# JeongsooP/RGB-no-more

Hardware: AMD Instinct MI355X
Metric: images/sec JPEG-Ti DCT 512x512 train step (higher is better)
Workload: dtype bf16

## Files before the change

rgb-no-more_amd/csrc/vit_chain_bwd.hip:

```cpp
#include "common.h"
#include <string.h>
#include <type_traits>
#include "internal.h"
#include "ln_bwd_rows.h"
#include "../../include/rgbnm.h"

namespace {

typedef __attribute__((address_space(3))) void* lds_ptr;
typedef const __attribute__((address_space(1))) void* glb_ptr;
typedef unsigned int u32x2 __attribute__((ext_vector_type(2)));
typedef unsigned int u32x4 __attribute__((ext_vector_type(4)));
typedef bf16 bf16x2v __attribute__((ext_vector_type(2)));

constexpr int E = 192, HID = 768, HD = 64, HEADS = 3, NTOK = 196, NTILE = 7, NPAD = 224, INNER = HEADS * HD, LDQ = 3 * INNER;
constexpr int NCW = 7, NTHREADS = 64 * (NCW + 1), CTHREADS = 64 * NCW, BM = 32 * NCW;
constexpr int ROWB = 128, ARR = NPAD * ROWB, SLOT = 24576, STAGE = 2 * SLOT, CH = 64, NCHUNK = HID / CH;
constexpr int CP = E + 4;
constexpr int SMEM = 163840;
#ifndef PIPE_P
#define PIPE_P 6
#endif
#ifndef PIPE_M1
#define PIPE_M1 5
#endif
#ifndef PIPE_X
#define PIPE_X 7
#endif
constexpr int M_STG = 2 * STAGE;
constexpr int TILE = 32 * ROWB;
typedef rgbnm::LnBwdRows<CTHREADS, BM> LnBwd;
constexpr int RED_OFF = (BM * CP * 2 + 1023) / 1024 * 1024;
static_assert(RED_OFF + LnBwd::RED_BYTES <= 132096, "LDS");
constexpr int P_SLOT0 = 132096, P_SLOT1 = 0, P_TILES = 98304;
static_assert(P_SLOT0 + SLOT <= SMEM && P_TILES + NCW * TILE <= P_SLOT0, "LDS");
constexpr int A_Q = 0, A_K = ARR, A_V = 2 * ARR, A_G = 3 * ARR, A_L2 = 4 * ARR, A_D = A_L2 + NPAD * 4, A_STG = A_D + NPAD * 4;
constexpr int STG_PITCH = 144, STG_WAVE = 32 * STG_PITCH;
constexpr int A_SIDE = A_STG + NCW * STG_WAVE;
static_assert(A_SIDE + NCW * 1024 <= SMEM, "LDS");
constexpr int X_SLOT0 = A_K, X_SLOT1 = A_K + SLOT, X_SLOT2 = 0, X_TILES = A_K + 2 * SLOT, X_TSET = NCW * TILE;
static_assert(X_SLOT1 + SLOT <= X_TILES && X_TILES + 3 * X_TSET <= SMEM && SLOT <= A_K, "LDS");

struct BwdBlk {
  const bf16* wimg;
  const float *ln1_g, *ln2_g;
  const bf16* x_in; const float *mean1, *rstd1;
  const bf16* qkv; const float* lse; const bf16* attn; const bf16* x_mid; const float *mean2, *rstd2; const bf16* gp;
  const bf16* dy;
  bf16* du; bf16* dx_mid; bf16* dqkv; bf16* dx;
  float *part2, *part1;
};
static_assert(sizeof(BwdBlk) == sizeof(rgbnm_chain_bwd_block), "rgbnm_chain_bwd_block layout");
constexpr int MAX_DEPTH = 12;
struct BwdArgs {
  BwdBlk blk[MAX_DEPTH]; bf16* dattn;
  int depth, nimg;
  float scale;
};

__device__ __forceinline__ int fswz(int row) {
  return (((row >> 1) & 1) << 2) | ((row >> 2) & 1) | (((row >> 3) & 1) << 1);
}
struct Geo {
  int lane, l31, g, fl;
  unsigned tr0;
};
__device__ __forceinline__ Geo make_geo() {
  Geo L;
  L.lane = threadIdx.x & 63;
  L.l31 = L.lane & 31;
  L.g = L.lane >> 5;
  L.fl = fswz(L.l31);
  const int k = (L.lane >> 2) & 3, G1 = (L.lane >> 4) & 1, l3 = L.lane & 3;
  const int pc = (2 * G1 + (l3 >> 1)) ^ (((k >> 1) << 2) | L.g);
  L.tr0 = (unsigned)((4 * L.g + k) * ROWB + pc * 16 + 8 * (l3 & 1));
  return L;
}
__device__ __forceinline__ Geo fresh_geo() {
  Geo L;
  L.lane = lane_id_here();
  L.l31 = L.lane & 31;
  L.g = L.lane >> 5;
  L.fl = fswz(L.l31);
  const int k = (L.lane >> 2) & 3, G1 = (L.lane >> 4) & 1, l3 = L.lane & 3;
  const int pc = (2 * G1 + (l3 >> 1)) ^ (((k >> 1) << 2) | L.g);
  L.tr0 = (unsigned)((4 * L.g + k) * ROWB + pc * 16 + 8 * (l3 & 1));
  return L;
}
template <int T> struct TileLoop {
// ... 46 lines not shown
#ifndef XB_ROWPIPE
#define XB_ROWPIPE 1
#endif
__device__ __forceinline__ void row_pair_mma(f32x16& sa, f32x16& da, const unsigned char* arrS, const unsigned char* arrD, unsigned rb,
                                             int t, const Frag<bf16> (&xs)[4], const Frag<bf16> (&xd)[4]) {
#if XB_ROWPIPE
#define XB_SB __builtin_amdgcn_sched_barrier(0)
  Frag<bf16> fs[4], fd[4];
  XB_SB;
  fs[0] = rowfrag_x(arrS, rb, t, 0);
  fd[0] = rowfrag_x(arrD, rb, t, 0);
  fs[1] = rowfrag_x(arrS, rb, t, 1);
  fd[1] = rowfrag_x(arrD, rb, t, 1);
  XB_SB;
  mma(sa, fs[0], xs[0]); XB_SB;
  fs[2] = rowfrag_x(arrS, rb, t, 2); XB_SB;
  mma(da, fd[0], xd[0]); XB_SB;
  fd[2] = rowfrag_x(arrD, rb, t, 2); XB_SB;
  mma(sa, fs[1], xs[1]); XB_SB;
  fs[3] = rowfrag_x(arrS, rb, t, 3); XB_SB;
  mma(da, fd[1], xd[1]); XB_SB;
  fd[3] = rowfrag_x(arrD, rb, t, 3); XB_SB;
  mma(sa, fs[2], xs[2]);
  mma(da, fd[2], xd[2]);
  mma(sa, fs[3], xs[3]);
  mma(da, fd[3], xd[3]);
  XB_SB;
#undef XB_SB
#else
#pragma unroll
  for (int c = 0; c < 4; ++c) {
    mma(sa, rowfrag_x(arrS, rb, t, c), xs[c]);
    mma(da, rowfrag_x(arrD, rb, t, c), xd[c]);
  }
#endif
}
__device__ __forceinline__ unsigned opaque(unsigned v) {
  asm volatile("" : "+v"(v));
  return v;
}
__device__ __forceinline__ void wg_barrier() {
  asm volatile("" ::: "memory");
  __builtin_amdgcn_s_barrier();
  asm volatile("" ::: "memory");
}
template <int N> __device__ __forceinline__ void wait_vm() { asm volatile("s_waitcnt vmcnt(%0)" ::"n"(N) : "memory"); }
__device__ __forceinline__ void wait_lds() { asm volatile("s_waitcnt lgkmcnt(0)" ::: "memory"); }
#ifndef XB_NT
#define XB_NT 1
#endif
#ifndef XB_NTLD
#define XB_NTLD 0
#endif
template <bool NT, typename V, typename P>
__device__ __forceinline__ void gstore(P* ptr, const V& v) {
#ifdef XB_NOSTORE
  if ((XB_NOSTORE & 1) && NT) return;
  if ((XB_NOSTORE & 2) && !NT) return;
#endif
  if constexpr (NT) __builtin_nontemporal_store(v, reinterpret_cast<V*>(ptr));
  else *reinterpret_cast<V*>(ptr) = v;
}

#ifdef X_LDSWAIT
__device__ __forceinline__ void own_tile_fence() { wait_lds(); }
#else
__device__ __forceinline__ void own_tile_fence() { asm volatile("" ::: "memory"); }
#endif
__device__ __forceinline__ unsigned pack2(float a, float b) {
  const bf16x2v v = {(bf16)a, (bf16)b};
  unsigned r = __builtin_bit_cast(unsigned, v);
  asm volatile("" : "+v"(r));
  return r;
}
__device__ __forceinline__ bf16x8 as_bf16x8(u32x4 v) { return __builtin_bit_cast(bf16x8, v); }
struct Rows { u32x4 v[12]; };

template <int NKB>
__device__ __forceinline__ void dma_linear(const unsigned char* src, unsigned char* dst, int lane) {
#pragma unroll
  for (int i = 0; i < NKB; ++i)
    __builtin_amdgcn_global_load_lds((glb_ptr)(src + i * 1024 + lane * 16), (lds_ptr)(dst + i * 1024), 16, 0, 0);
}
__device__ __forceinline__ void dma_matrix_all(const bf16* __restrict__ src, int ld, unsigned char* dst, int lane) {
#pragma unroll 4
  for (int i = 0; i < 28; ++i) {
    const int row = 8 * i + (lane >> 3), pc = lane & 7;
    const int lc = pc ^ fswz(row);
    const int srow = row < NTOK ? row : NTOK - 1;
    __builtin_amdgcn_global_load_lds((glb_ptr)(src + (size_t)srow * ld + lc * 8), (lds_ptr)(dst + i * 1024), 16, 0, (XB_NTLD & 2) ? 2 : 0);
  }
}
__device__ __forceinline__ void dma_row_tiles(const bf16* __restrict__ src, int ld, unsigned char* dst, int lane) {
#pragma unroll 4
  for (int i = 0; i < 28; ++i) {
    const int row = 8 * i + (lane >> 3), pc = lane & 7;
    const int lc = pc ^ (row & 7);
    const int srow = row < NTOK ? row : NTOK - 1;
    __builtin_amdgcn_global_load_lds((glb_ptr)(src + (size_t)srow * ld + lc * 8), (lds_ptr)(dst + i * 1024), 16, 0, 0);
  }
}

__device__ __forceinline__ void tile_out(unsigned char* smem, unsigned stg, const u32x4& p0, const u32x4& p1, const u32x4& p2,
                                         const u32x4& p3, bf16* dst, int ld, int live) {
  const int ln = lane_id_here();
  const unsigned wo = stg + (unsigned)((ln & 31) * ROWB + (((ln >> 5) ^ (ln & 7)) << 4));
  *reinterpret_cast<u32x4*>(smem + wo) = p0;
  *reinterpret_cast<u32x4*>(smem + (wo ^ 32u)) = p1;
  *reinterpret_cast<u32x4*>(smem + (wo ^ 64u)) = p2;
  *reinterpret_cast<u32x4*>(smem + (wo ^ 96u)) = p3;
  own_tile_fence();
  const int rl = ln >> 3, seg = ln & 7;
  const unsigned ro = stg + (unsigned)(rl * ROWB + ((seg ^ rl) << 4));
  bf16* gp = dst + (size_t)rl * ld + seg * 8;
  u32x4 v[4];
#pragma unroll
  for (int i = 0; i < 4; ++i) v[i] = *reinterpret_cast<const u32x4*>(smem + ro + i * 8 * ROWB);
  if (live == 32) {
#pragma unroll
    for (int i = 0; i < 4; ++i) gstore<(XB_NT & 4) != 0>(gp + (size_t)i * 8 * ld, v[i]);
  } else {
#pragma unroll
    for (int i = 0; i < 4; ++i)
      if (i * 8 + rl < live) gstore<(XB_NT & 4) != 0>(gp + (size_t)i * 8 * ld, v[i]);
  }
  own_tile_fence();
}

__device__ __forceinline__ void gemm_k192(f32x16& acc, const unsigned char* sW, int ht, const Rows& x, const Geo& L) {
  int wbase = L.l31 * (E * 2) + ((L.g ^ L.fl) << 4) + ht * 32 * (E * 2);
  asm volatile("" : "+v"(wbase));
#pragma unroll
  for (int c = 0; c < 12; ++c) {
    Frag<bf16> fb, fx;
    fb.v = *reinterpret_cast<const bf16x8*>(sW + ((wbase ^ ((c % 4) << 5)) + 128 * (c / 4)));
    fx.v = as_bf16x8(x.v[c]);
    mma(acc, fb, fx);
  }
}

template <int DEPTH>
__device__ __forceinline__ void gemm_k192x2(f32x16& a0, f32x16& a1, const unsigned char* sW, const Rows& x, const Geo& L) {
  int wb0 = L.l31 * (E * 2) + ((L.g ^ L.fl) << 4);
  asm volatile("" : "+v"(wb0));
  const int wb1 = wb0 + 32 * (E * 2);
  Frag<bf16> fb[24];
#pragma unroll
  for (int i = 0; i < 24; ++i) {
    const int c = i >> 1;
    fb[i].v = *reinterpret_cast<const bf16x8*>(sW + ((((i & 1) ? wb1 : wb0) ^ ((c % 4) << 5)) + 128 * (c / 4)));
  }
#pragma unroll
  for (int i = 0; i < 24; ++i) {
    Frag<bf16> fx;
    fx.v = as_bf16x8(x.v[i >> 1]);
    mma((i & 1) ? a1 : a0, fb[i], fx);
  }
  __builtin_amdgcn_sched_group_barrier(0x100, DEPTH, 0);
#pragma unroll
  for (int i = 0; i < 24 - DEPTH; ++i) {
    __builtin_amdgcn_sched_group_barrier(0x008, 1, 0);
    __builtin_amdgcn_sched_group_barrier(0x100, 1, 0);
  }
#pragma unroll
  for (int i = 0; i < DEPTH; ++i) __builtin_amdgcn_sched_group_barrier(0x008, 1, 0);
  __builtin_amdgcn_sched_barrier(0);
}
typedef bf16 bf16x4v __attribute__((ext_vector_type(4)));
typedef __attribute__((address_space(3))) bf16x4v* lds_b64_ptr;
__device__ __forceinline__ u32x2 tr_read(const unsigned char* smem, unsigned off) {
// ... 39 lines not shown
      v[wv][i] = PRIVATE ? *reinterpret_cast<const u32x4*>(src + wv * STG_WAVE + r * STG_PITCH + seg * 16)
                         : *reinterpret_cast<const u32x4*>(src + (wv * 32 + r) * ROWB + ((seg ^ (r & 7)) << 4));
    }
}
__device__ __forceinline__ void tiles_write(const u32x4 (&v)[NTILE][4], bf16* __restrict__ g0, size_t ld, int lane) {
  const int rl = lane >> 3, seg = lane & 7;
#pragma unroll
  for (int wv = 0; wv < NTILE; ++wv)
#pragma unroll
    for (int i = 0; i < 4; ++i) {
      const int row = wv * 32 + i * 8 + rl;
      if (row < NTOK) gstore<(XB_NT & 2) != 0>(g0 + (size_t)row * ld + seg * 8, v[wv][i]);
    }
}

#ifdef CHAINB_PROF
__device__ unsigned long long g_chainb_prof[8 * 8 * 128];
#define CP_(i)                                                                                          \
  do {                                                                                                  \
    if (ib == CHAINB_PROF_BLK && blockIdx.x < 8) {                                                      \
      const unsigned long long t_ = __builtin_amdgcn_s_memtime();                                       \
      if ((threadIdx.x & 63) == 0) g_chainb_prof[(blockIdx.x * 8 + (threadIdx.x >> 6)) * 128 + (i)] = t_; \
    }                                                                                                   \
  } while (0)
#ifndef CHAINB_PROF_BLK
#define CHAINB_PROF_BLK 6
#endif
#else
#define CP_(i) do {} while (0)
#endif
#define BAR(s) do { CP_(2 * (s)); wg_barrier(); CP_(2 * (s) + 1); } while (0)
constexpr int B_M0 = 0;
constexpr int B_E2 = 12;
constexpr int B_P = 19;
constexpr int B_A = 24;
constexpr int B_X = 37;
constexpr int B_E1 = 46;
constexpr int B_END = 53;

__device__ __forceinline__ void ln_bwd_request(LnBwd& lnb, const bf16* X, const float* mean, const float* rstd, const bf16* R, int img,
                                               int w) {
  const int tid = w * 64 + lane_id_here();
  lnb.request_x(X, E, mean, rstd, img * NTOK, NTOK, tid);
  lnb.request_res(R, E, img * NTOK, NTOK, tid);
}
template <int B0>
__device__ __forceinline__ void ln_bwd_epilogue(unsigned char* smem, const f32x16 (&acc)[6], const bf16* X, const float* mean,
                                                const float* rstd, const bf16* R, const float* gamma, bf16* DX,
                                                float* part, int img, int w, int ib) {
  const int lane_ = lane_id_here();
  const int tid = w * 64 + lane_, rloc = w * 32 + (lane_ & 31), g = lane_ >> 5;
  LnBwd lnb;
  lnb.request_x(X, E, mean, rstd, img * NTOK, NTOK, tid);
  lnb.request_res(R, E, img * NTOK, NTOK, tid);
  wait_lds();
  BAR(B0);
  bf16* Cs = reinterpret_cast<bf16*>(smem);
#pragma unroll
  for (int b = 0; b < 6; ++b)
#pragma unroll
    for (int q = 0; q < 4; ++q) {
      const int nl = 32 * b + 8 * q + 4 * g;
      const f32x4 v = {acc[b][4 * q + 0], acc[b][4 * q + 1], acc[b][4 * q + 2], acc[b][4 * q + 3]};
      store4<bf16>(Cs + rloc * CP + nl, v);
    }
  wait_lds();
  BAR(B0 + 1);
  lnb.run<true>(Cs, CP, DX, E, gamma, true, part, img, reinterpret_cast<float*>(smem + RED_OFF), img * NTOK, NTOK, tid, Cs,
          [&](int k) { if (k == 0) BAR(B0 + 2); else if (k == 1) BAR(B0 + 3); else if (k == 2) BAR(B0 + 4); else BAR(B0 + 5); });
  wait_lds();
  BAR(B0 + 6);
}
__device__ __forceinline__ void read_own_rows(const unsigned char* smem, int w, Rows& x) {
  const int lane_ = lane_id_here();
  const unsigned char* rp = smem + (w * 32 + (lane_ & 31)) * (CP * 2) + 16 * (lane_ >> 5);
#pragma unroll
  for (int c = 0; c < 12; ++c) {
    const u32x2 lo = *reinterpret_cast<const u32x2*>(rp + 32 * c), hi = *reinterpret_cast<const u32x2*>(rp + 32 * c + 8);
    x.v[c] = u32x4{lo[0], lo[1], hi[0], hi[1]};
  }
}

__global__ __launch_bounds__(NTHREADS) void vit_chain_bwd_kernel(BwdArgs p) {
  extern __shared__ __attribute__((aligned(16))) unsigned char smem[];
  const int img = blockIdx.x;
  if (img >= p.nimg) return;
  const int w = __builtin_amdgcn_readfirstlane(threadIdx.x >> 6);
  const int depth = p.depth;

  if (w == NCW) {
#ifdef X_DMAPRIO
    __builtin_amdgcn_s_setprio(X_DMAPRIO);
#endif
    const int lane = threadIdx.x & 63;
    for (int ib = depth - 1; ib >= 0; --ib) {
      const BwdBlk& b = p.blk[ib];
      const unsigned char* wimg = reinterpret_cast<const unsigned char*>(b.wimg);
      dma_linear<48>(wimg, smem, lane);
      for (int c = 0; c < NCHUNK; ++c) {
        wait_vm<0>();
        BAR(B_M0 + c);
        if (c + 1 < NCHUNK) dma_linear<48>(wimg + (size_t)(c + 1) * STAGE, smem + ((c + 1) & 1) * STAGE, lane);
      }
      BAR(B_E2);
      dma_linear<24>(wimg + (size_t)NCHUNK * STAGE, smem + P_SLOT0, lane);
#pragma unroll
      for (int k = 1; k < 7; ++k) BAR(B_E2 + k);
      const bf16* qkv0 = b.qkv + (size_t)img * NTOK * LDQ;
      const bf16* do0 = p.dattn + (size_t)img * NTOK * INNER;
      bf16* dq0 = b.dqkv + (size_t)img * NTOK * LDQ;
      const unsigned char* stg0 = smem + A_STG;
      auto issue_kv = [&](int h) {
        dma_matrix_all(qkv0 + INNER + h * HD, LDQ, smem + A_K, lane);
        dma_matrix_all(qkv0 + 2 * INNER + h * HD, LDQ, smem + A_V, lane);
      };
      auto issue_q = [&](int h) { dma_matrix_all(qkv0 + h * HD, LDQ, smem + A_Q, lane); };
      auto issue_g = [&](int h) { dma_matrix_all(do0 + h * HD, INNER, smem + A_G, lane); };
      const unsigned char* xw = wimg + (size_t)NCHUNK * STAGE + 3 * SLOT;
      auto issue_xt = [&](int j) { dma_row_tiles(dq0 + j * 64, LDQ, smem + X_TILES + (j % 3) * X_TSET, lane); };
      wait_vm<0>();
      BAR(B_P);
      BAR(B_P + 1);
      dma_linear<24>(wimg + (size_t)NCHUNK * STAGE + SLOT, smem + P_SLOT1, lane);
      issue_kv(0);
      wait_vm<56>(); BAR(B_P + 2);
      dma_linear<24>(wimg + (size_t)NCHUNK * STAGE + 2 * SLOT, smem + P_SLOT0, lane);
      wait_vm<0>(); BAR(B_P + 3);
      issue_q(0);
      BAR(B_P + 4);
      {
        issue_g(0);
        wait_vm<0>();
        BAR(B_A);
        for (int h = 0; h < HEADS; ++h) {
          bf16* g0 = dq0 + h * HD;
          wait_vm<0>();
          BAR(B_A + 1 + 4 * h);
          u32x4 tq[NTILE][4];
          tiles_read<true>(stg0, lane, tq);
          wait_lds();
          BAR(B_A + 2 + 4 * h);
          tiles_write(tq, g0, LDQ, lane);
          if (h + 1 < HEADS) issue_kv(h + 1);
          else {
            dma_linear<24>(xw, smem + X_SLOT0, lane);
            dma_linear<24>(xw + SLOT, smem + X_SLOT1, lane);
          }
          wait_vm<0>();
          BAR(B_A + 3 + 4 * h);
          tiles_read<true>(stg0, lane, tq);
          wait_lds();
          BAR(B_A + 4 + 4 * h);
          tiles_write(tq, g0 + INNER, LDQ, lane);
          tiles_read<false>(smem + A_G, lane, tq);
          wait_lds();
          if (h + 1 < HEADS) {
            issue_q(h + 1);
            issue_g(h + 1);
          } else {
            issue_xt(0);
          }
          tiles_write(tq, g0 + 2 * INNER, LDQ, lane);
        }
      }
      for (int j = 0; j < 9; ++j) {
        if (j == 0) wait_vm<28>();
        else if (j + 1 < 9) wait_vm<52>();
        else wait_vm<0>();
        BAR(B_X + j);
        if (j == 0) {
          issue_xt(1);
          dma_linear<24>(xw + 2 * SLOT, smem + X_SLOT2, lane);
          issue_xt(2);
        }
        if (j + 2 < 9 && j >= 1) {
          dma_linear<24>(xw + (size_t)(j + 2) * SLOT, smem + ((j + 2) % 3 == 0 ? X_SLOT0 : ((j + 2) % 3 == 1 ? X_SLOT1 : X_SLOT2)), lane);
          issue_xt(j + 2);
        }
      }
#pragma unroll
      for (int k = 0; k < 7; ++k) BAR(B_E1 + k);
      BAR(B_END);
    }
    return;
  }

#if defined(X_PRIO) && X_PRIO == 1
  if (w >= 4) __builtin_amdgcn_s_setprio(1);
#elif defined(X_PRIO) && X_PRIO == 2
  if (w < 4) __builtin_amdgcn_s_setprio(1);
#endif
  const int row0 = 32 * w;
  const int live = NTOK - row0 < 32 ? NTOK - row0 : 32;
  const size_t grow0 = (size_t)img * NTOK + row0;
  const float LOG2E = 1.4426950408889634f;
  const float c2 = p.scale * LOG2E;

  Rows dyf;
  {
    const int lane_ = lane_id_here();
    const int rloc = row0 + (lane_ & 31), tok = rloc < NTOK ? rloc : NTOK - 1;
    const bf16* yrow = p.blk[depth - 1].dy + ((size_t)img * NTOK + tok) * E + 8 * (lane_ >> 5);
#pragma unroll
    for (int c = 0; c < 12; ++c) dyf.v[c] = *reinterpret_cast<const u32x4*>(yrow + 16 * c);
  }

  for (int ib = depth - 1; ib >= 0; --ib) {
    const BwdBlk& b = p.blk[ib];
    f32x16 acc2[6];
#pragma unroll
    for (int bt = 0; bt < 6; ++bt)
#pragma unroll
      for (int r = 0; r < 16; ++r) acc2[bt][r] = 0.f;
    {
      const Geo L = fresh_geo();
      const int fl = L.fl;
      const int woff0 = L.l31 * (E * 2) + ((L.g ^ fl) << 4);
      const unsigned stg = (unsigned)(M_STG + w * 2 * TILE);
      bf16x8 gpraw[4];
      auto load_gp = [&](int chunk) {
        const int ln = lane_id_here();
#pragma unroll
        for (int i = 0; i < 4; ++i) {
          const int idx = ln + 64 * i, row = idx >> 3, vec = idx & 7;
          int rr = row0 + row;
          rr = rr < NTOK ? rr : NTOK - 1;
          const bf16x8* gsrc = reinterpret_cast<const bf16x8*>(b.gp + ((size_t)img * NTOK + rr) * HID + chunk * CH + vec * 8);
          gpraw[i] = (XB_NTLD & 1) ? __builtin_nontemporal_load(gsrc) : *gsrc;
        }
      };
      load_gp(0);
      for (int chunk = 0; chunk < NCHUNK; ++chunk) {
// ... 75 lines not shown
            for (int bt = 0; bt < 6; ++bt)
              fw[bt].v = *reinterpret_cast<const bf16x8*>(smem + (w2o ^ (unsigned)(s << 5)) + bt * 32 * ROWB);
#pragma unroll
            for (int bt = 0; bt < 6; ++bt) mma(acc2[bt], fw[bt], pg[hs]);
          }
#else
          __builtin_amdgcn_sched_barrier(0);
#pragma unroll
          for (int bt = 0; bt < 6; ++bt)
            fw2[6 + bt].v = *reinterpret_cast<const bf16x8*>(smem + (w2o ^ (unsigned)((2 * ht + 1) << 5)) + bt * 32 * ROWB);
#pragma unroll
          for (int bt = 0; bt < 6; ++bt) mma(acc2[bt], fw2[bt], pg[0]);
#pragma unroll
          for (int bt = 0; bt < 6; ++bt) mma(acc2[bt], fw2[6 + bt], pg[1]);
#pragma unroll
          for (int i = 0; i < 6; ++i) {
            __builtin_amdgcn_sched_group_barrier(0x008, 1, 0);
            __builtin_amdgcn_sched_group_barrier(0x100, 1, 0);
          }
          __builtin_amdgcn_sched_group_barrier(0x008, 6, 0);
          __builtin_amdgcn_sched_barrier(0);
#endif
        }
        own_tile_fence();
        const int ln = lane_id_here();
        bf16x8 dv0[4];
#pragma unroll
        for (int i = 0; i < 4; ++i) {
          const int idx = ln + 64 * i, row = idx >> 3, vec = idx & 7;
          dv0[i] = *reinterpret_cast<const bf16x8*>(smem + stg + TILE + row * ROWB + ((vec ^ (row & 7)) << 4));
        }
        if (live == 32) {
#pragma unroll
          for (int i = 0; i < 4; ++i) {
            const int idx = ln + 64 * i, row = idx >> 3, vec = idx & 7;
            gstore<(XB_NT & 1) != 0>(b.du + (grow0 + row) * HID + chunk * CH + vec * 8, dv0[i]);
          }
        } else {
#pragma unroll
          for (int i = 0; i < 4; ++i) {
            const int idx = ln + 64 * i, row = idx >> 3, vec = idx & 7;
            if (row < live) gstore<(XB_NT & 1) != 0>(b.du + (grow0 + row) * HID + chunk * CH + vec * 8, dv0[i]);
          }
        }
      }
    }
    ln_bwd_epilogue<B_E2>(smem, acc2, b.x_mid, b.mean2, b.rstd2, b.dy, b.ln2_g, b.dx_mid, b.part2, img, w, ib);
    {
      const Geo L = fresh_geo();
      Rows dxf;
      read_own_rows(smem, w, dxf);
      wait_lds();
      BAR(B_P);
      const unsigned stg = (unsigned)(P_TILES + w * TILE);
#pragma unroll
      for (int h = 0; h < HEADS; ++h) {
        BAR(B_P + 1 + h);
        const unsigned char* sW = smem + (h == 1 ? P_SLOT1 : P_SLOT0);
        f32x16 acc[2];
#pragma unroll
        for (int ht = 0; ht < 2; ++ht)
#pragma unroll
          for (int r = 0; r < 16; ++r) acc[ht][r] = 0.f;
#ifdef X_NOPIPE
        gemm_k192(acc[0], sW, 0, dxf, L);
        gemm_k192(acc[1], sW, 1, dxf, L);
#else
        gemm_k192x2<PIPE_P>(acc[0], acc[1], sW, dxf, L);
#endif
        u32x4 pc[4];
#pragma unroll
        for (int ht = 0; ht < 2; ++ht)
#pragma unroll
          for (int hs = 0; hs < 2; ++hs)
#pragma unroll
            for (int d = 0; d < 4; ++d) pc[2 * ht + hs][d] = pack2(acc[ht][8 * hs + 2 * d], acc[ht][8 * hs + 2 * d + 1]);
        tile_out(smem, stg, pc[0], pc[1], pc[2], pc[3], p.dattn + grow0 * INNER + h * HD, INNER, live);
      }
      asm volatile("s_waitcnt vmcnt(0)" ::: "memory");
      BAR(B_P + 4);
    }
    {
      unsigned char* Qs = smem + A_Q;
      unsigned char* Ks = smem + A_K;
      unsigned char* Vs = smem + A_V;
      unsigned char* Gs = smem + A_G;
      float* L2_s = reinterpret_cast<float*>(smem + A_L2);
      float* D_s = reinterpret_cast<float*>(smem + A_D);
      unsigned char* stg = smem + A_STG + w * STG_WAVE;
      const Geo L = fresh_geo();
      const int fl = L.fl;
      const unsigned rb0 = (unsigned)(L.l31 * ROWB + ((L.g ^ fl) << 4));
      const int row = row0 + L.l31;
      u32x4 qraw[4], graw[4], oraw[4];
      float lq = 0.f;
      const bf16* qkv0 = b.qkv + (size_t)img * NTOK * LDQ;
      const bf16* do0 = p.dattn + (size_t)img * NTOK * INNER;
      const bf16* o0 = b.attn + (size_t)img * NTOK * INNER;
      auto load_own_g = [&](int h) {
        const int lane_ = lane_id_here();
        const int seg = lane_ & 7;
#pragma unroll
        for (int i = 0; i < 4; ++i) {
          int r = row0 + i * 8 + (lane_ >> 3);
          r = r < NTOK ? r : NTOK - 1;
          graw[i] = *reinterpret_cast<const u32x4*>(do0 + (size_t)r * INNER + h * HD + seg * 8);
        }
      };
      unsigned char* qside = smem + A_SIDE + w * 1024;
      auto load_own_q = [&](int h) {
        const int lane_ = lane_id_here();
        const int seg = lane_ & 7;
#pragma unroll
        for (int i = 0; i < 4; ++i) {
          int r = row0 + i * 8 + (lane_ >> 3);
          r = r < NTOK ? r : NTOK - 1;
          const bf16* src = qkv0 + (size_t)r * LDQ + h * HD + seg * 8;
          if (i == 0) __builtin_amdgcn_global_load_lds((glb_ptr)src, (lds_ptr)qside, 16, 0, 0);
          else qraw[i] = *reinterpret_cast<const u32x4*>(src);
        }
      };
      auto load_own_o = [&](int h) {
        const int lane_ = lane_id_here();
        const int seg = lane_ & 7;
#pragma unroll
        for (int i = 0; i < 4; ++i) {
          int r = row0 + i * 8 + (lane_ >> 3);
          r = r < NTOK ? r : NTOK - 1;
          oraw[i] = *reinterpret_cast<const u32x4*>(o0 + (size_t)r * INNER + h * HD + seg * 8);
        }
        int rq_ = row0 + (lane_ & 31);
        rq_ = rq_ < NTOK ? rq_ : NTOK - 1;
        lq = b.lse[((size_t)img * HEADS + h) * NTOK + rq_];
      };
      load_own_g(0);
      load_own_q(0);
      load_own_o(0);
      BAR(B_A);
      for (int h = 0; h < HEADS; ++h) {
        const bool more = h + 1 < HEADS;
        asm volatile("s_waitcnt vmcnt(0)" ::: "memory");
        Frag<bf16> kf[4], vf[4];
        {
          f32x16 dq[2];
          Frag<bf16> qf[4], gf[4];
          const int rl = L.lane >> 3, seg = L.lane & 7;
#pragma unroll
          for (int i = 0; i < 4; ++i) {
            const bf16x8 gv = __builtin_bit_cast(bf16x8, graw[i]), ov = __builtin_bit_cast(bf16x8, oraw[i]);
            float d = 0.f;
#pragma unroll
            for (int e = 0; e < 8; ++e) d += (float)gv[e] * (float)ov[e];
            d += lane_xor1(d);
            d += lane_xor2(d);
            d += lane_xor4(d);
            if (seg == 0) D_s[row0 + i * 8 + rl] = d;
          }
          qraw[0] = *reinterpret_cast<const u32x4*>(qside + lane_id_here() * 16);
#pragma unroll
          for (int i = 0; i < 4; ++i) *reinterpret_cast<u32x4*>(stg + (i * 8 + rl) * STG_PITCH + seg * 16) = qraw[i];
          own_tile_fence();
#pragma unroll
          for (int c = 0; c < 4; ++c) qf[c].v = *reinterpret_cast<const bf16x8*>(stg + L.l31 * STG_PITCH + (2 * c + L.g) * 16);
          own_tile_fence();
#pragma unroll
          for (int i = 0; i < 4; ++i) *reinterpret_cast<u32x4*>(stg + (i * 8 + rl) * STG_PITCH + seg * 16) = graw[i];
          own_tile_fence();
#pragma unroll
          for (int c = 0; c < 4; ++c) gf[c].v = *reinterpret_cast<const bf16x8*>(stg + L.l31 * STG_PITCH + (2 * c + L.g) * 16);
          const float Dq = D_s[row];
          own_tile_fence();
          const float lq2 = lq * LOG2E;
          if (L.g == 0) L2_s[row] = lq2;
#pragma unroll
          for (int dt = 0; dt < 2; ++dt)
#pragma unroll
            for (int r = 0; r < 16; ++r) dq[dt][r] = 0.f;
          unsigned rb = rb0, tr = L.tr0;
          asm volatile("" : "+v"(rb), "+v"(tr));
          const unsigned kt = (unsigned)A_K + tr;
          TileLoop<NTILE>::run([&](auto tc) {
            constexpr int t = decltype(tc)::value;
            f32x16 sa, da;
#pragma unroll
            for (int r = 0; r < 16; ++r) { sa[r] = 0.f; da[r] = 0.f; }
            row_pair_mma(sa, da, Ks, Vs, rb, t, qf, gf);
            float ds[16];
#pragma unroll
// ... 41 lines not shown
            for (int r = 0; r < 16; ++r) { sa[r] = 0.f; da[r] = 0.f; }
            row_pair_mma(sa, da, Qs, Gs, rb, t, kf, vf);
            float pp[16], ds[16];
#pragma unroll
            for (int q4 = 0; q4 < 4; ++q4) {
              const f32x4 l4 = *reinterpret_cast<const f32x4*>(L2_s + t * 32 + 8 * q4 + 4 * L.g);
              const f32x4 d4 = *reinterpret_cast<const f32x4*>(D_s + t * 32 + 8 * q4 + 4 * L.g);
#pragma unroll
              for (int e = 0; e < 4; ++e) {
                const int r = 4 * q4 + e;
                const float pr = __builtin_amdgcn_exp2f(fmaf(sa[r], c2, -l4[e]));
                pp[r] = pr;
                ds[r] = pr * (da[r] - d4[e]);
              }
            }
            if (t * 32 + 32 > NTOK) {
#pragma unroll
              for (int r = 0; r < 16; ++r)
                if (t * 32 + acc_row(r, L.lane) >= NTOK) { pp[r] = 0.f; ds[r] = 0.f; }
            }
            Frag<bf16> gg[4];
            tfrag4<t>(gt_, gg);
            Frag<bf16> f = pfrag(pp, 0);
            mma(dv[0], gg[0], f);
            mma(dv[1], gg[1], f);
            f = pfrag(pp, 1);
            mma(dv[0], gg[2], f);
            mma(dv[1], gg[3], f);
            tfrag4<t>(qt_, gg);
            f = pfrag(ds, 0);
            mma(dk[0], gg[0], f);
            mma(dk[1], gg[1], f);
            f = pfrag(ds, 1);
            mma(dk[0], gg[2], f);
            mma(dk[1], gg[3], f);
          });
          if (more) load_own_g(h + 1);
          tile_park_private(stg, dk, p.scale, L);
          if (more) load_own_q(h + 1);
          wait_lds();
          BAR(B_A + 3 + 4 * h);
          tile_park_rows(Gs, w, dv, 1.0f);
        }
        if (more) load_own_o(h + 1);
        wait_lds();
        BAR(B_A + 4 + 4 * h);
      }
    }
    f32x16 accx[6];
#pragma unroll
    for (int bt = 0; bt < 6; ++bt)
#pragma unroll
      for (int r = 0; r < 16; ++r) accx[bt][r] = 0.f;
    for (int j = 0; j < 9; ++j) {
      BAR(B_X + j);
      const Geo L = fresh_geo();
      const int fl = L.fl;
      const int set = j % 3;
      const unsigned wo = opaque((unsigned)((set == 0 ? X_SLOT0 : (set == 1 ? X_SLOT1 : X_SLOT2)) + L.l31 * ROWB + ((L.g ^ fl) << 4)));
      const unsigned to = opaque((unsigned)(X_TILES + set * X_TSET + w * TILE + L.l31 * ROWB + ((L.g ^ (L.l31 & 7)) << 4)));
#pragma unroll
      for (int s = 0; s < 4; ++s) {
        Frag<bf16> fx, fw[6];
        fx.v = *reinterpret_cast<const bf16x8*>(smem + (to ^ (unsigned)(s << 5)));
#pragma unroll
        for (int bt = 0; bt < 6; ++bt)
          fw[bt].v = *reinterpret_cast<const bf16x8*>(smem + (wo ^ (unsigned)(s << 5)) + bt * 32 * ROWB);
#pragma unroll
        for (int bt = 0; bt < 6; ++bt) mma(accx[bt], fw[bt], fx);
      }
#ifndef X_NOPIPE
      __builtin_amdgcn_sched_group_barrier(0x100, PIPE_X, 0);
#pragma unroll
      for (int i = 0; i < 24; ++i) {
        __builtin_amdgcn_sched_group_barrier(0x008, 1, 0);
        if (i < 28 - PIPE_X) __builtin_amdgcn_sched_group_barrier(0x100, 1, 0);
      }
      __builtin_amdgcn_sched_barrier(0);
#endif
    }
    ln_bwd_epilogue<B_E1>(smem, accx, b.x_in, b.mean1, b.rstd1, b.dx_mid, b.ln1_g, b.dx, b.part1, img, w, ib);
    read_own_rows(smem, w, dyf);
    wait_lds();
    BAR(B_END);
  }
}

}

#ifdef CHAINB_PROF
extern "C" int rgbnm_chainb_prof_read(unsigned long long* host_out) {
  return hipMemcpyFromSymbol(host_out, HIP_SYMBOL(g_chainb_prof), sizeof(unsigned long long) * 8 * 8 * 128) == hipSuccess ? 0 : -1;
}
#endif

extern "C" {

size_t rgbnm_chain_bwd_block_bytes(void) { return sizeof(BwdBlk); }

int rgbnm_vit_chain_bwd(const rgbnm_vit_cfg* c, const rgbnm_chain_bwd_block* blocks, int depth, void* dattn, void* stream) {
  if (!c || !blocks || !dattn || depth <= 0) return RGBNM_EINVAL;
  if (c->dtype != RGBNM_DT_BF16 || c->E != E || c->heads != HEADS || c->N != NTOK || c->B < 1 || depth > MAX_DEPTH) return 1;
  BwdArgs p;
  memcpy(p.blk, blocks, sizeof(BwdBlk) * depth);
  p.dattn = (bf16*)dattn; p.depth = depth; p.nimg = c->B; p.scale = c->attn_scale;
  static DevOnce attr;
  if (attr.need()) {
    if (hipFuncSetAttribute((const void*)vit_chain_bwd_kernel, hipFuncAttributeMaxDynamicSharedMemorySize, SMEM) != hipSuccess)
// ... 15 lines not shown
```

rgb-no-more_amd/csrc/common.h:

```cpp
#pragma once
#include <hip/hip_runtime.h>
#include <stdint.h>

typedef __bf16 bf16;
typedef bf16 bf16x8 __attribute__((ext_vector_type(8)));
typedef bf16 bf16x4 __attribute__((ext_vector_type(4)));
typedef _Float16 f16;
typedef f16 f16x8 __attribute__((ext_vector_type(8)));
typedef f16 f16x4 __attribute__((ext_vector_type(4)));
typedef float f32x16 __attribute__((ext_vector_type(16)));
typedef float f32x4 __attribute__((ext_vector_type(4)));

#if (defined(X_NOLN) || defined(X_NOGELU) || defined(X_NOEXP) || defined(X_NOSAVE) || defined(X_HALFW) || defined(X_NOATTN) || \
     defined(X_NOMLP) || defined(X_NOPIPE) || defined(KPX_NOGELU) || defined(KPX_NOC2) || defined(KPX_NOSTORE)) &&             \
    !defined(RGBNM_EXPERIMENTS)
#error "a wrong-numbers timing switch (X_NO* / X_HALFW / KPX_NO*) is defined without -DRGBNM_EXPERIMENTS"
#endif

#define RGBNM_OK 0
#define RGBNM_EINVAL (-1)
#define RGBNM_ELAUNCH (-2)
#define RGBNM_EWORKSPACE (-3)

enum { DT_F32 = 0, DT_BF16 = 1, DT_F16 = 2 };

#include <atomic>
struct DevOnce {
  std::atomic<unsigned long long> mask{0};
  static int dev() { int d = 0; (void)hipGetDevice(&d); return d & 63; }
  bool need() const { return !((mask.load(std::memory_order_acquire) >> dev()) & 1ULL); }
  void done() { mask.fetch_or(1ULL << dev(), std::memory_order_release); }
};

#define LAUNCH_CHECK()                                  \
  do {                                                  \
    hipError_t e__ = hipGetLastError();                 \
    if (e__ != hipSuccess) return RGBNM_ELAUNCH;        \
  } while (0)

template <typename T> struct Frag;
template <> struct Frag<bf16> {
  bf16x8 v;
  static constexpr int EPL = 8;
};
template <> struct Frag<f16> {
  f16x8 v;
  static constexpr int EPL = 8;
};
template <> struct Frag<float> {
  f32x4 v;
  static constexpr int EPL = 4;
};

__device__ __forceinline__ void mma(f32x16& acc, const Frag<bf16>& a, const Frag<bf16>& b) {
  acc = __builtin_amdgcn_mfma_f32_32x32x16_bf16(a.v, b.v, acc, 0, 0, 0);
}
__device__ __forceinline__ void mma(f32x16& acc, const Frag<f16>& a, const Frag<f16>& b) {
  acc = __builtin_amdgcn_mfma_f32_32x32x16_f16(a.v, b.v, acc, 0, 0, 0);
}
__device__ __forceinline__ void mma(f32x16& acc, const Frag<float>& a, const Frag<float>& b) {
#pragma unroll
  for (int j = 0; j < 4; ++j) acc = __builtin_amdgcn_mfma_f32_32x32x2f32(a.v[j], b.v[j], acc, 0, 0, 0);
}

__device__ __forceinline__ int acc_row(int r, int lane) { return (r & 3) + 8 * (r >> 2) + 4 * (lane >> 5); }

template <typename T> __device__ __forceinline__ Frag<T> load_frag(const T* p);
template <> __device__ __forceinline__ Frag<bf16> load_frag<bf16>(const bf16* p) {
  Frag<bf16> f;
// ... 186 lines not shown
```

Baseline: 67630.

## Keep head-0 dattn tile in LDS for attention backward instead of reloading

Moves the P-phase staging tiles so the head-0 dattn output can be written straight into the A_G LDS region with the attention-phase swizzle. The attention backward then reads its first gradient rows from LDS rather than reloading them from global memory via DMA, which removes a global round trip and a wait at the phase boundary. It also adds an optional (off by default) path where compute waves DMA their own dqkv row tiles for the X phase. The LDS layout changes (P_SLOT0 moves to the end, tile 6 is relocated), and padding rows are filled by replicating the last live row, so correctness depends on the new static asserts and on region lifetimes not overlapping.

```diff
diff --git a/rgb-no-more_amd/csrc/vit_chain_bwd.hip b/rgb-no-more_amd/csrc/vit_chain_bwd.hip
--- a/rgb-no-more_amd/csrc/vit_chain_bwd.hip
+++ b/rgb-no-more_amd/csrc/vit_chain_bwd.hip
@@ -32,9 +32,17 @@
 typedef rgbnm::LnBwdRows<CTHREADS, BM> LnBwd;
 constexpr int RED_OFF = (BM * CP * 2 + 1023) / 1024 * 1024;
 static_assert(RED_OFF + LnBwd::RED_BYTES <= 132096, "LDS");
-constexpr int P_SLOT0 = 132096, P_SLOT1 = 0, P_TILES = 98304;
+constexpr int A_Q = 0, A_K = ARR, A_V = 2 * ARR, A_G = 3 * ARR, A_L2 = 4 * ARR, A_D = A_L2 + NPAD * 4, A_STG = A_D + NPAD * 4;
+#ifndef XB_DO0
+#define XB_DO0 1
+#endif
+#if XB_DO0
+constexpr int P_SLOT0 = SMEM - SLOT, P_SLOT1 = 0, P_TILES = A_L2, P_TILE6 = SLOT;
+static_assert(P_TILES + 6 * TILE <= P_SLOT0 && P_TILE6 + TILE <= A_K && A_G + ARR <= P_TILES && RED_OFF + LnBwd::RED_BYTES <= P_SLOT0, "LDS");
+#else
+constexpr int P_SLOT0 = 132096, P_SLOT1 = 0, P_TILES = 98304, P_TILE6 = P_TILES + 6 * TILE;
 static_assert(P_SLOT0 + SLOT <= SMEM && P_TILES + NCW * TILE <= P_SLOT0, "LDS");
-constexpr int A_Q = 0, A_K = ARR, A_V = 2 * ARR, A_G = 3 * ARR, A_L2 = 4 * ARR, A_D = A_L2 + NPAD * 4, A_STG = A_D + NPAD * 4;
+#endif
 constexpr int STG_PITCH = 144, STG_WAVE = 32 * STG_PITCH;
 constexpr int A_SIDE = A_STG + NCW * STG_WAVE;
 static_assert(A_SIDE + NCW * 1024 <= SMEM, "LDS");
@@ -235,22 +243,40 @@
     __builtin_amdgcn_global_load_lds((glb_ptr)(src + (size_t)srow * ld + lc * 8), (lds_ptr)(dst + i * 1024), 16, 0, 0);
   }
 }
-
+__device__ __forceinline__ void dma_own_row_tile(const bf16* __restrict__ src, int ld, unsigned char* dst, int lane, int w) {
+#pragma unroll
+  for (int k = 0; k < 4; ++k) {
+    const int i = 4 * w + k;
+    const int row = 8 * i + (lane >> 3), pc = lane & 7;
+    const int lc = pc ^ (row & 7);
+    const int srow = row < NTOK ? row : NTOK - 1;
+    __builtin_amdgcn_global_load_lds((glb_ptr)(src + (size_t)srow * ld + lc * 8), (lds_ptr)(dst + i * 1024), 16, 0, 0);
+  }
+}
+#ifndef XB_XOWN
+#define XB_XOWN 0
+#endif
+
+template <bool AG = false>
 __device__ __forceinline__ void tile_out(unsigned char* smem, unsigned stg, const u32x4& p0, const u32x4& p1, const u32x4& p2,
                                          const u32x4& p3, bf16* dst, int ld, int live) {
   const int ln = lane_id_here();
-  const unsigned wo = stg + (unsigned)((ln & 31) * ROWB + (((ln >> 5) ^ (ln & 7)) << 4));
+  const unsigned wo = stg + (unsigned)((ln & 31) * ROWB + (((ln >> 5) ^ (AG ? fswz(ln & 31) : (ln & 7))) << 4));
   *reinterpret_cast<u32x4*>(smem + wo) = p0;
   *reinterpret_cast<u32x4*>(smem + (wo ^ 32u)) = p1;
   *reinterpret_cast<u32x4*>(smem + (wo ^ 64u)) = p2;
   *reinterpret_cast<u32x4*>(smem + (wo ^ 96u)) = p3;
   own_tile_fence();
   const int rl = ln >> 3, seg = ln & 7;
-  const unsigned ro = stg + (unsigned)(rl * ROWB + ((seg ^ rl) << 4));
   bf16* gp = dst + (size_t)rl * ld + seg * 8;
   u32x4 v[4];
 #pragma unroll
-  for (int i = 0; i < 4; ++i) v[i] = *reinterpret_cast<const u32x4*>(smem + ro + i * 8 * ROWB);
+  for (int i = 0; i < 4; ++i)
+    v[i] = *reinterpret_cast<const u32x4*>(smem + stg + (i * 8 + rl) * ROWB + ((seg ^ (AG ? fswz(i * 8 + rl) : rl)) << 4));
+  if (AG && live < 32) {
+    const u32x4 last = *reinterpret_cast<const u32x4*>(smem + stg + (live - 1) * ROWB + ((seg ^ fswz(live - 1)) << 4));
+    for (int r = live + rl; r < 32; r += 8) *reinterpret_cast<u32x4*>(smem + stg + r * ROWB + ((seg ^ fswz(r)) << 4)) = last;
+  }
   if (live == 32) {
 #pragma unroll
     for (int i = 0; i < 4; ++i) gstore<(XB_NT & 4) != 0>(gp + (size_t)i * 8 * ld, v[i]);
@@ -469,6 +495,13 @@
       issue_kv(0);
       wait_vm<56>(); BAR(B_P + 2);
       dma_linear<24>(wimg + (size_t)NCHUNK * STAGE + 2 * SLOT, smem + P_SLOT0, lane);
+#if XB_DO0
+      wait_vm<0>(); BAR(B_P + 3);
+      BAR(B_P + 4);
+      {
+        BAR(B_A);
+        issue_q(0);
+#else
       wait_vm<0>(); BAR(B_P + 3);
       issue_q(0);
       BAR(B_P + 4);
@@ -476,6 +509,7 @@
         issue_g(0);
         wait_vm<0>();
         BAR(B_A);
+#endif
         for (int h = 0; h < HEADS; ++h) {
           bf16* g0 = dq0 + h * HD;
           wait_vm<0>();
@@ -507,6 +541,16 @@
           tiles_write(tq, g0 + 2 * INNER, LDQ, lane);
         }
       }
+#if XB_XOWN
+      for (int j = 0; j < 9; ++j) {
+        if (j == 0) wait_vm<28>();
+        else if (j + 1 < 9) wait_vm<24>();
+        else wait_vm<0>();
+        BAR(B_X + j);
+        if (j + 2 < 9)
+          dma_linear<24>(xw + (size_t)(j + 2) * SLOT, smem + ((j + 2) % 3 == 0 ? X_SLOT0 : ((j + 2) % 3 == 1 ? X_SLOT1 : X_SLOT2)), lane);
+      }
+#else
       for (int j = 0; j < 9; ++j) {
         if (j == 0) wait_vm<28>();
         else if (j + 1 < 9) wait_vm<52>();
@@ -522,6 +566,7 @@
           issue_xt(j + 2);
         }
       }
+#endif
 #pragma unroll
       for (int k = 0; k < 7; ++k) BAR(B_E1 + k);
       BAR(B_END);
@@ -703,7 +748,7 @@
       read_own_rows(smem, w, dxf);
       wait_lds();
       BAR(B_P);
-      const unsigned stg = (unsigned)(P_TILES + w * TILE);
+      const unsigned stg = (unsigned)(w < 6 ? P_TILES + w * TILE : P_TILE6);
 #pragma unroll
       for (int h = 0; h < HEADS; ++h) {
         BAR(B_P + 1 + h);
@@ -726,9 +771,16 @@
           for (int hs = 0; hs < 2; ++hs)
 #pragma unroll
             for (int d = 0; d < 4; ++d) pc[2 * ht + hs][d] = pack2(acc[ht][8 * hs + 2 * d], acc[ht][8 * hs + 2 * d + 1]);
-        tile_out(smem, stg, pc[0], pc[1], pc[2], pc[3], p.dattn + grow0 * INNER + h * HD, INNER, live);
+        if (XB_DO0 && h == 0)
+          tile_out<true>(smem, (unsigned)(A_G + row0 * ROWB), pc[0], pc[1], pc[2], pc[3], p.dattn + grow0 * INNER, INNER, live);
+        else
+          tile_out(smem, stg, pc[0], pc[1], pc[2], pc[3], p.dattn + grow0 * INNER + h * HD, INNER, live);
       }
+#if XB_DO0
+      wait_lds();
+#else
       asm volatile("s_waitcnt vmcnt(0)" ::: "memory");
+#endif
       BAR(B_P + 4);
     }
     {
@@ -784,7 +836,19 @@
         rq_ = rq_ < NTOK ? rq_ : NTOK - 1;
         lq = b.lse[((size_t)img * HEADS + h) * NTOK + rq_];
       };
+#if XB_DO0
+      {
+        const int lane_ = lane_id_here();
+        const int seg = lane_ & 7;
+#pragma unroll
+        for (int i = 0; i < 4; ++i) {
+          const int r = row0 + i * 8 + (lane_ >> 3);
+          graw[i] = *reinterpret_cast<const u32x4*>(Gs + r * ROWB + ((seg ^ fswz(r)) << 4));
+        }
+      }
+#else
       load_own_g(0);
+#endif
       load_own_q(0);
       load_own_o(0);
       BAR(B_A);
@@ -932,8 +996,25 @@
     for (int bt = 0; bt < 6; ++bt)
 #pragma unroll
       for (int r = 0; r < 16; ++r) accx[bt][r] = 0.f;
+#if XB_XOWN
+    const bf16* dqw = b.dqkv + (size_t)img * NTOK * LDQ;
+#endif
     for (int j = 0; j < 9; ++j) {
       BAR(B_X + j);
+#if XB_XOWN
+      {
+        const int lane_ = lane_id_here();
+        if (j == 0) {
+          dma_own_row_tile(dqw + 64, LDQ, smem + X_TILES + X_TSET, lane_, w);
+          dma_own_row_tile(dqw + 128, LDQ, smem + X_TILES + 2 * X_TSET, lane_, w);
+        } else {
+          if (j + 2 < 9) dma_own_row_tile(dqw + (j + 2) * 64, LDQ, smem + X_TILES + ((j + 2) % 3) * X_TSET, lane_, w);
+          if (j + 2 < 9) wait_vm<8>();
+          else if (j + 1 < 9) wait_vm<4>();
+          else wait_vm<0>();
+        }
+      }
+#endif
       const Geo L = fresh_geo();
       const int fl = L.fl;
       const int set = j % 3;
```

Measured after the change: 67800 (median of 6 runs). About the same (+0.2%).

## Compute head-0 attention gradient last and keep it in LDS instead of global round trip

Applied to the files above, without the earlier changes.

Reorders the per-head dattn projection so head 0 is computed last (head order 1,2,0), loading weight slots accordingly. Head 0's result is written directly into the swizzled A_G LDS array rather than stored to global and re-read by the DMA wave and compute waves, removing a global write/read round trip for that head. It also adds X_NORR experiment switches that skip residual/g/xt loads for timing studies, guarded by the experiments check. The risk is LDS aliasing between A_G and other live buffers, plus an extra LDS wait before the barrier.

```diff
diff --git a/rgb-no-more_amd/csrc/common.h b/rgb-no-more_amd/csrc/common.h
--- a/rgb-no-more_amd/csrc/common.h
+++ b/rgb-no-more_amd/csrc/common.h
@@ -12,9 +12,9 @@
 typedef float f32x4 __attribute__((ext_vector_type(4)));
 
 #if (defined(X_NOLN) || defined(X_NOGELU) || defined(X_NOEXP) || defined(X_NOSAVE) || defined(X_HALFW) || defined(X_NOATTN) || \
-     defined(X_NOMLP) || defined(X_NOPIPE) || defined(KPX_NOGELU) || defined(KPX_NOC2) || defined(KPX_NOSTORE)) &&             \
+     defined(X_NOMLP) || defined(X_NOPIPE) || defined(X_NORR) || defined(KPX_NOGELU) || defined(KPX_NOC2) || defined(KPX_NOSTORE)) &&             \
     !defined(RGBNM_EXPERIMENTS)
-#error "a wrong-numbers timing switch (X_NO* / X_HALFW / KPX_NO*) is defined without -DRGBNM_EXPERIMENTS"
+#error "a wrong-numbers timing switch (X_NO* / X_NORR / X_HALFW / KPX_NO*) is defined without -DRGBNM_EXPERIMENTS"
 #endif
 
 #define RGBNM_OK 0
diff --git a/rgb-no-more_amd/csrc/vit_chain_bwd.hip b/rgb-no-more_amd/csrc/vit_chain_bwd.hip
--- a/rgb-no-more_amd/csrc/vit_chain_bwd.hip
+++ b/rgb-no-more_amd/csrc/vit_chain_bwd.hip
@@ -34,6 +34,7 @@
 static_assert(RED_OFF + LnBwd::RED_BYTES <= 132096, "LDS");
 constexpr int P_SLOT0 = 132096, P_SLOT1 = 0, P_TILES = 98304;
 static_assert(P_SLOT0 + SLOT <= SMEM && P_TILES + NCW * TILE <= P_SLOT0, "LDS");
+__device__ __forceinline__ constexpr int P_HEAD(int s) { return s == 2 ? 0 : s + 1; }
 constexpr int A_Q = 0, A_K = ARR, A_V = 2 * ARR, A_G = 3 * ARR, A_L2 = 4 * ARR, A_D = A_L2 + NPAD * 4, A_STG = A_D + NPAD * 4;
 constexpr int STG_PITCH = 144, STG_WAVE = 32 * STG_PITCH;
 constexpr int A_SIDE = A_STG + NCW * STG_WAVE;
@@ -187,6 +188,14 @@
 #ifndef XB_NTLD
 #define XB_NTLD 0
 #endif
+#ifndef X_NORR
+#define X_NORR 0
+#endif
+template <typename T> __device__ __forceinline__ T opaque_undef() {
+  T v;
+  asm volatile("" : "=v"(v));
+  return v;
+}
 template <bool NT, typename V, typename P>
 __device__ __forceinline__ void gstore(P* ptr, const V& v) {
 #ifdef XB_NOSTORE
@@ -396,7 +405,14 @@
   const int tid = w * 64 + lane_, rloc = w * 32 + (lane_ & 31), g = lane_ >> 5;
   LnBwd lnb;
   lnb.request_x(X, E, mean, rstd, img * NTOK, NTOK, tid);
+#if X_NORR & 4
+#pragma unroll
+  for (int it = 0; it < LnBwd::ITERS; ++it)
+#pragma unroll
+    for (int v = 0; v < 3; ++v) lnb.lr[it][v] = opaque_undef<bf16x8>();
+#else
   lnb.request_res(R, E, img * NTOK, NTOK, tid);
+#endif
   wait_lds();
   BAR(B0);
   bf16* Cs = reinterpret_cast<bf16*>(smem);
@@ -447,7 +463,7 @@
         if (c + 1 < NCHUNK) dma_linear<48>(wimg + (size_t)(c + 1) * STAGE, smem + ((c + 1) & 1) * STAGE, lane);
       }
       BAR(B_E2);
-      dma_linear<24>(wimg + (size_t)NCHUNK * STAGE, smem + P_SLOT0, lane);
+      dma_linear<24>(wimg + (size_t)(NCHUNK * STAGE + P_HEAD(0) * SLOT), smem + P_SLOT0, lane);
 #pragma unroll
       for (int k = 1; k < 7; ++k) BAR(B_E2 + k);
       const bf16* qkv0 = b.qkv + (size_t)img * NTOK * LDQ;
@@ -459,21 +475,20 @@
         dma_matrix_all(qkv0 + 2 * INNER + h * HD, LDQ, smem + A_V, lane);
       };
       auto issue_q = [&](int h) { dma_matrix_all(qkv0 + h * HD, LDQ, smem + A_Q, lane); };
-      auto issue_g = [&](int h) { dma_matrix_all(do0 + h * HD, INNER, smem + A_G, lane); };
+      auto issue_g = [&](int h) { if (!(X_NORR & 1)) dma_matrix_all(do0 + h * HD, INNER, smem + A_G, lane); };
       const unsigned char* xw = wimg + (size_t)NCHUNK * STAGE + 3 * SLOT;
-      auto issue_xt = [&](int j) { dma_row_tiles(dq0 + j * 64, LDQ, smem + X_TILES + (j % 3) * X_TSET, lane); };
+      auto issue_xt = [&](int j) { if (!(X_NORR & 2)) dma_row_tiles(dq0 + j * 64, LDQ, smem + X_TILES + (j % 3) * X_TSET, lane); };
       wait_vm<0>();
       BAR(B_P);
       BAR(B_P + 1);
-      dma_linear<24>(wimg + (size_t)NCHUNK * STAGE + SLOT, smem + P_SLOT1, lane);
+      dma_linear<24>(wimg + (size_t)(NCHUNK * STAGE + P_HEAD(1) * SLOT), smem + P_SLOT1, lane);
       issue_kv(0);
       wait_vm<56>(); BAR(B_P + 2);
-      dma_linear<24>(wimg + (size_t)NCHUNK * STAGE + 2 * SLOT, smem + P_SLOT0, lane);
+      dma_linear<24>(wimg + (size_t)(NCHUNK * STAGE + P_HEAD(2) * SLOT), smem + P_SLOT0, lane);
       wait_vm<0>(); BAR(B_P + 3);
       issue_q(0);
       BAR(B_P + 4);
       {
-        issue_g(0);
         wait_vm<0>();
         BAR(B_A);
         for (int h = 0; h < HEADS; ++h) {
@@ -705,9 +720,10 @@
       BAR(B_P);
       const unsigned stg = (unsigned)(P_TILES + w * TILE);
 #pragma unroll
-      for (int h = 0; h < HEADS; ++h) {
-        BAR(B_P + 1 + h);
-        const unsigned char* sW = smem + (h == 1 ? P_SLOT1 : P_SLOT0);
+      for (int st = 0; st < HEADS; ++st) {
+        const int h = P_HEAD(st);
+        BAR(B_P + 1 + st);
+        const unsigned char* sW = smem + (st == 1 ? P_SLOT1 : P_SLOT0);
         f32x16 acc[2];
 #pragma unroll
         for (int ht = 0; ht < 2; ++ht)
@@ -726,9 +742,16 @@
           for (int hs = 0; hs < 2; ++hs)
 #pragma unroll
             for (int d = 0; d < 4; ++d) pc[2 * ht + hs][d] = pack2(acc[ht][8 * hs + 2 * d], acc[ht][8 * hs + 2 * d + 1]);
-        tile_out(smem, stg, pc[0], pc[1], pc[2], pc[3], p.dattn + grow0 * INNER + h * HD, INNER, live);
+        if (h != 0) {
+          tile_out(smem, stg, pc[0], pc[1], pc[2], pc[3], p.dattn + grow0 * INNER + h * HD, INNER, live);
+        } else {
+          unsigned char* gr = smem + A_G + (row0 + L.l31) * ROWB;
+#pragma unroll
+          for (int k = 0; k < 4; ++k) *reinterpret_cast<u32x4*>(gr + (((2 * k + L.g) ^ L.fl) << 4)) = pc[k];
+        }
       }
       asm volatile("s_waitcnt vmcnt(0)" ::: "memory");
+      wait_lds();
       BAR(B_P + 4);
     }
     {
@@ -755,7 +778,7 @@
         for (int i = 0; i < 4; ++i) {
           int r = row0 + i * 8 + (lane_ >> 3);
           r = r < NTOK ? r : NTOK - 1;
-          graw[i] = *reinterpret_cast<const u32x4*>(do0 + (size_t)r * INNER + h * HD + seg * 8);
+          graw[i] = (X_NORR & 1) ? opaque_undef<u32x4>() : *reinterpret_cast<const u32x4*>(do0 + (size_t)r * INNER + h * HD + seg * 8);
         }
       };
       unsigned char* qside = smem + A_SIDE + w * 1024;
@@ -784,7 +807,15 @@
         rq_ = rq_ < NTOK ? rq_ : NTOK - 1;
         lq = b.lse[((size_t)img * HEADS + h) * NTOK + rq_];
       };
-      load_own_g(0);
+      {
+        const int lane_ = lane_id_here();
+        const int seg = lane_ & 7;
+#pragma unroll
+        for (int i = 0; i < 4; ++i) {
+          const int r = row0 + i * 8 + (lane_ >> 3);
+          graw[i] = *reinterpret_cast<const u32x4*>(Gs + r * ROWB + ((seg ^ fswz(r)) << 4));
+        }
+      }
       load_own_q(0);
       load_own_o(0);
       BAR(B_A);
```

After: 66400 before, 66800 after, median of 6. About the same (+0.6%).
